# MrBottleTree/fake-video-detection-engine

Hardware: NVIDIA B200
Metric: 1080p_keyframes_per_sec_v5_ela_texture (higher is better)
Workload: dtype int32

## Files before the change

### fake-video-detection-engine_b200/csrc/v5ela_device.cuh

```cuda
#pragma once
#include <stdint.h>
#include <string.h>

#include "v5ela.h"

#ifdef __CUDACC__
#define V5_DEV __device__ __forceinline__
#define V5_HOSTDEV __host__ __device__ __forceinline__
#else
#define V5_DEV inline
#define V5_HOSTDEV inline
#endif

#ifndef V5_NS
#define V5_NS v5
#endif

namespace v5plan {

#ifndef V5_NT
#define V5_NT 256
#endif
#ifndef V5_TW_MAX
#define V5_TW_MAX 30
// ... 460 lines not shown
V5_DEV int neg_cr_of(const uint32_t *w, int k)
{
    return rgb_dot<false, -32768, 27439, 5329>(w, k, 65535 - ((128 << 16) + 32767)) >> 16;
}

template <bool WANT_Y, bool WANT_C>
V5_DEV void convert8x2(const uint8_t *la, const uint8_t *lb, U2 &y0, U2 &y1, uint32_t &cbo, uint32_t &cro)
{
    uint32_t a[6], b[6];
#pragma unroll
    for (int i = 0; i < 3; i++) {
        const U2 ta = reinterpret_cast<const U2 *>(la)[i], tb = reinterpret_cast<const U2 *>(lb)[i];
        a[2 * i] = ta.x; a[2 * i + 1] = ta.y;
        b[2 * i] = tb.x; b[2 * i + 1] = tb.y;
    }
    if (WANT_Y) {
        int ya[8], yb[8];
#pragma unroll
        for (int k = 0; k < 8; k++) {
            ya[k] = y_of(a, k);
            yb[k] = y_of(b, k);
        }
        y0 = U2{pack4sat(ya[0], ya[1], ya[2], ya[3]), pack4sat(ya[4], ya[5], ya[6], ya[7])};
        y1 = U2{pack4sat(yb[0], yb[1], yb[2], yb[3]), pack4sat(yb[4], yb[5], yb[6], yb[7])};
    }
    if (WANT_C) {
        int c[4], d[4];
#pragma unroll
        for (int j = 0; j < 4; j++) {
            const int bias = 1 + (j & 1);
            c[j] = (bias - (neg_cb_of(a, 2 * j) + neg_cb_of(a, 2 * j + 1) + neg_cb_of(b, 2 * j) + neg_cb_of(b, 2 * j + 1))) >> 2;
            d[j] = (bias - (neg_cr_of(a, 2 * j) + neg_cr_of(a, 2 * j + 1) + neg_cr_of(b, 2 * j) + neg_cr_of(b, 2 * j + 1))) >> 2;
        }
        cbo = pack4sat(c[0], c[1], c[2], c[3]);
        cro = pack4sat(d[0], d[1], d[2], d[3]);
    }
}

V5_DEV void convert_wait_done(int tid, Smem &S, const KParams &p, const Geo &g, int r, ThreadAcc &acc, bool prefetch_next)
{
    mbar_wait(reinterpret_cast<uint64_t *>(&S.done_bar), (acc.phase >> 2) & 1u);
    acc.phase ^= 4u;
    if (prefetch_next) stage_prefetch(tid, S, p, g, r + 1);
}

V5_DEV void stage_convert(int tid, Smem &S, const KParams &p, const Geo &g, int r, ThreadAcc &acc, bool defer, bool prefetch_next, bool copy_carry = true)
{
    const int last_cline = ((g.h + 1) >> 1) - 1 - 8 * r;
    const int last_line = g.h - 1 - 16 * r;
    const uint8_t(*src)[RGB_PITCH] = S.rgb[rb(r)];
    bool waiting = defer;
    if (RGB_BUFS == 2 && !waiting && copy_carry)
        for (int i = tid; i < RGB_PITCH / 16; i += NT)
            reinterpret_cast<U4 *>(S.rgb_carry[r & 1])[i] = reinterpret_cast<const U4 *>(src[15])[i];
#if defined(V5_CONVERT_UNROLL) && V5_CONVERT_UNROLL
#pragma unroll 2
#endif
    for (int u = tid; u < 8 * 2 * BAND_MCUS; u += NT) {
        const int li = u / (2 * BAND_MCUS), ox = u - li * (2 * BAND_MCUS);
        const int mcu = g.m0 - 1 + (ox >> 1);
        if (ox >= 2 * g.band_mcus || mcu < 0 || mcu >= g.mw) continue;
        U2 y0, y1;
        uint32_t cb, cr;
        convert8x2<true, true>(&src[2 * li][24 * ox], &src[2 * li + 1][24 * ox], y0, y1, cb, cr);
        const int jc = li < last_cline ? li : last_cline;
        int lb = 2 * jc + 1;
        if (lb > last_line) lb = last_line;
        if (jc != li || lb != 2 * li + 1) {
            U2 d0, d1;
            convert8x2<false, true>(&src[2 * jc][24 * ox], &src[lb][24 * ox], d0, d1, cb, cr);
        }
        if (waiting) {
            convert_wait_done(tid, S, p, g, r, acc, prefetch_next);
            waiting = false;
            if (RGB_BUFS == 2)
                for (int i = tid; i < RGB_PITCH / 16; i += NT)
                    reinterpret_cast<U4 *>(S.rgb_carry[r & 1])[i] = reinterpret_cast<const U4 *>(src[15])[i];
        }
        *reinterpret_cast<U2 *>(&S.yorig[ring16(r, 2 * li)][8 * ox]) = y0;
        *reinterpret_cast<U2 *>(&S.yorig[ring16(r, 2 * li + 1)][8 * ox]) = y1;
        *reinterpret_cast<uint32_t *>(&S.cenc[0][li][4 * ox]) = cb;
        *reinterpret_cast<uint32_t *>(&S.cenc[1][li][4 * ox]) = cr;
    }
    if (waiting) {
        convert_wait_done(tid, S, p, g, r, acc, prefetch_next);
        if (RGB_BUFS == 2)
            for (int i = tid; i < RGB_PITCH / 16; i += NT)
                reinterpret_cast<U4 *>(S.rgb_carry[r & 1])[i] = reinterpret_cast<const U4 *>(src[15])[i];
    }
}

V5_DEV void stage_carries(int tid, Smem &S, int r, bool has_band)
{
    constexpr int NRGB = RGB_PITCH / 16, NY = Y_PITCH / 16;
    if (tid < NRGB) {
        if (has_band) reinterpret_cast<U4 *>(S.rgb_carry[r & 1])[tid] = reinterpret_cast<const U4 *>(S.rgb[rb(r)][15])[tid];
    } else if (FUSE2_OK && tid < NRGB + 2 * NY) {
        const int k = tid - NRGB, line = k >= NY ? 1 : 0, i = k - line * NY;
        reinterpret_cast<U4 *>(S.ycarry[FUSE2_OK ? line : 0])[FUSE2_OK ? i : 0] = reinterpret_cast<const U4 *>(S.yorig[ring16(r - 1, 14 + line)])[i];
    }
}

#define V5_C0_298 2446
#define V5_C0_390 3196
#define V5_C0_541 4433
#define V5_C0_765 6270
#define V5_C0_899 7373
#define V5_C1_175 9633
#define V5_C1_501 12299
#define V5_C1_847 15137
#define V5_C1_961 16069
#define V5_C2_053 16819
#define V5_C2_562 20995
#define V5_C3_072 25172

template <int S, bool PASS1>
V5_DEV void fdct8(int *v)
{
    const int n = PASS1 ? 11 : 15, rnd = 1 << (n - 1);
    const int t0 = v[0] + v[7 * S], t7 = v[0] - v[7 * S], t1 = v[S] + v[6 * S], t6 = v[S] - v[6 * S];
    const int t2 = v[2 * S] + v[5 * S], t5 = v[2 * S] - v[5 * S], t3 = v[3 * S] + v[4 * S], t4 = v[3 * S] - v[4 * S];
    const int t10 = t0 + t3, t13 = t0 - t3, t11 = t1 + t2, t12 = t1 - t2;
    if (PASS1) {
        v[0] = (t10 + t11 - 1024) * 4;
        v[4 * S] = (t10 - t11) * 4;
    } else {
        v[0] = (t10 + t11 + 2) >> 2;
        v[4 * S] = (t10 - t11 + 2) >> 2;
    }
    v[2 * S] = (t12 * V5_C0_541 + t13 * (V5_C0_541 + V5_C0_765) + rnd) >> n;
    v[6 * S] = (t13 * V5_C0_541 + t12 * (V5_C0_541 - V5_C1_847) + rnd) >> n;
    const int z1 = (t4 + t7) * -V5_C0_899, z2 = (t5 + t6) * -V5_C2_562;
    const int z3 = t4 + t6, z4 = t5 + t7;
    const int z5 = (z3 + z4) * V5_C1_175 + rnd;
    const int z3b = z3 * -V5_C1_961 + z5, z4b = z4 * -V5_C0_390 + z5;
    v[7 * S] = (t4 * V5_C0_298 + z1 + z3b) >> n;
    v[5 * S] = (t5 * V5_C2_053 + z2 + z4b) >> n;
    v[3 * S] = (t6 * V5_C3_072 + z2 + z3b) >> n;
    v[S] = (t7 * V5_C1_501 + z1 + z4b) >> n;
}

template <int S, bool FINAL>
V5_DEV void idct8(int *v)
{
    const int n = FINAL ? 18 : 11;
    const int rnd = (1 << (n - 1)) + (FINAL ? (128 << 18) : 0);
    const int i2 = v[2 * S], i6 = v[6 * S];
    const int t2 = i2 * V5_C0_541 + i6 * (V5_C0_541 - V5_C1_847);
    const int t3 = i6 * V5_C0_541 + i2 * (V5_C0_541 + V5_C0_765);
    const int t0 = (v[0] + v[4 * S]) * 8192 + rnd, t1 = (v[0] - v[4 * S]) * 8192 + rnd;
    int u0 = v[7 * S], u1 = v[5 * S], u2 = v[3 * S], u3 = v[S];
    const int z1 = (u0 + u3) * -V5_C0_899, z2 = (u1 + u2) * -V5_C2_562;
    const int z3 = u0 + u2, z4 = u1 + u3;
    const int z5 = (z3 + z4) * V5_C1_175;
    const int z3b = z3 * -V5_C1_961 + z5, z4b = z4 * -V5_C0_390 + z5;
    u0 = u0 * V5_C0_298 + z1 + z3b;
    u1 = u1 * V5_C2_053 + z2 + z4b;
    u2 = u2 * V5_C3_072 + z2 + z3b;
    u3 = u3 * V5_C1_501 + z1 + z4b;
    v[0] = (t0 + t3 + u3) >> n;
    v[7 * S] = (t0 + t3 - u3) >> n;
    v[S] = (t1 + t2 + u2) >> n;
    v[6 * S] = (t1 + t2 - u2) >> n;
    v[2 * S] = (t1 - t2 + u1) >> n;
    v[5 * S] = (t1 - t2 - u1) >> n;
    v[3 * S] = (t0 - t3 + u0) >> n;
    v[4 * S] = (t0 - t3 - u0) >> n;
}

V5_DEV uint32_t pack_s16(int lo, int hi)
{
#ifndef __CUDACC__
    if (lo < -32768 || lo > 32767 || hi < -32768 || hi > 32767) range_violations()++;
#endif
    return prmt((uint32_t)lo, (uint32_t)hi, 0x5410u);
}
V5_DEV int s16_lo(uint32_t w) { return (int)prmt(w, 0u, 0x9910u); }
V5_DEV int s16_hi(uint32_t w) { return (int)w >> 16; }

#if !V5_MMA_BLOCKS
struct BlockTask {
    const QEntry *q;
    const uint8_t *in;
    uint8_t *out;
    int pitch;
    bool active;
};

template <bool FAST>
V5_DEV BlockTask block_task(int blk, Smem &S, const KParams &p, const Geo &g, int r, bool want_y)
{
    BlockTask t;
    t.active = false;
    t.q = S.qtab[0];
    t.in = nullptr;
    t.out = nullptr;
    t.pitch = 0;
    const int tw = g.m1 - g.m0;
    const int nl = want_y ? 4 * tw : 0;
    if (blk < nl) {
        const int br = blk >= 2 * tw ? 1 : 0, bc = blk - br * 2 * tw;
        if (16 * r + 8 * br >= g.h || (!FAST && 16 * g.m0 + 8 * bc >= g.w)) return t;
        const int row = ring16(r, 8 * br), col = 16 + 8 * bc;
        t.in = &S.yorig[row][col];
        t.out = &S.ydec[ringd(r, 8 * br)][col];
        t.pitch = Y_PITCH;
        t.active = true;
    } else {
        const int c = blk - nl;
        if (c >= 2 * g.band_mcus) return t;
        const int comp = c >= g.band_mcus ? 1 : 0, cbk = c - comp * g.band_mcus;
        const int mcu = g.m0 - 1 + cbk;
        if (mcu < 0 || mcu >= g.mw) return t;
        t.q = S.qtab[1];
        t.in = &S.cenc[comp][0][8 * cbk];
        t.out = &S.cdec[comp][ring8(r, 0)][8 * cbk];
        t.pitch = C_PITCH;
        t.active = true;
    }
    return t;
}

template <bool FAST>
V5_DEV BlockTask block_task_of(int tid, Smem &S, const KParams &p, const Geo &g, int r, bool want_y, int round)
{
    return block_task<FAST>(round * (NT / 4) + (tid >> 5) * 8 + ((tid & 31) >> 2), S, p, g, r, want_y);
}

V5_DEV int blocks_in_band(const Geo &g, bool want_y) { return (want_y ? 4 * (g.m1 - g.m0) : 0) + 2 * g.band_mcus; }


V5_DEV void blocks_rows_fwd(int tid, Smem &S, const BlockTask &t)
{
    const int warp = tid >> 5, lane = tid & 31, j = lane & 3, bw = lane >> 2;
    if (!t.active) return;
    int a[8], b[8];
    const U2 wa = *reinterpret_cast<const U2 *>(t.in + (2 * j) * t.pitch);
    const U2 wb = *reinterpret_cast<const U2 *>(t.in + (2 * j + 1) * t.pitch);
#pragma unroll
    for (int k = 0; k < 4; k++) {
        a[k] = (int)byte_of(wa.x, k); a[4 + k] = (int)byte_of(wa.y, k);
        b[k] = (int)byte_of(wb.x, k); b[4 + k] = (int)byte_of(wb.y, k);
    }
    fdct8<1, true>(a);
    fdct8<1, true>(b);
    uint32_t *ts = &S.tscratch[warp][36 * bw];
#pragma unroll
    for (int c = 0; c < 8; c++) ts[4 * c + j] = pack_s16(a[c], b[c]);
}

V5_DEV void blocks_cols(int tid, Smem &S, const BlockTask &t, int *col)
{
    const int warp = tid >> 5, lane = tid & 31, j = lane & 3, bw = lane >> 2;
    if (!t.active) return;
    const uint32_t *ts = &S.tscratch[warp][36 * bw];
    const U4 w0 = *reinterpret_cast<const U4 *>(ts + 8 * j), w1 = *reinterpret_cast<const U4 *>(ts + 8 * j + 4);
    int a[8] = {s16_lo(w0.x), s16_hi(w0.x), s16_lo(w0.y), s16_hi(w0.y), s16_lo(w0.z), s16_hi(w0.z), s16_lo(w0.w), s16_hi(w0.w)};
    int b[8] = {s16_lo(w1.x), s16_hi(w1.x), s16_lo(w1.y), s16_hi(w1.y), s16_lo(w1.z), s16_hi(w1.z), s16_lo(w1.w), s16_hi(w1.w)};
    fdct8<1, false>(a);
    fdct8<1, false>(b);
    const QEntry *qj = t.q + 2 * j;
#pragma unroll
    for (int k = 0; k < 8; k++) {
        const QEntry ea = qj[8 * k], eb = qj[8 * k + 1];
        const uint32_t xa = (uint32_t)(a[k] + (a[k] >> 31) + ea.bias), xb = (uint32_t)(b[k] + (b[k] >> 31) + eb.bias);
        a[k] = (int)umulhi32(xa, ea.recip) * ea.t - ea.unbias;
        b[k] = (int)umulhi32(xb, eb.recip) * eb.t - eb.unbias;
    }
    idct8<1, false>(a);
    idct8<1, false>(b);
#pragma unroll
    for (int k = 0; k < 8; k++) {
        col[k] = a[k];
        col[8 + k] = b[k];
    }
}

V5_DEV void blocks_cols_store(int tid, Smem &S, const BlockTask &t, const int *col)
{
    const int warp = tid >> 5, lane = tid & 31, j = lane & 3, bw = lane >> 2;
    if (!t.active) return;
    uint32_t *rs = &S.tscratch[warp][36 * bw];
#pragma unroll
    for (int k = 0; k < 8; k++) rs[4 * k + j] = pack_s16(col[k], col[8 + k]);
}

V5_DEV void blocks_rows_inv(int tid, Smem &S, const BlockTask &t)
{
    const int warp = tid >> 5, lane = tid & 31, j = lane & 3, bw = lane >> 2;
    if (!t.active) return;
    const uint32_t *rs = &S.tscratch[warp][36 * bw];
    const U4 w0 = *reinterpret_cast<const U4 *>(rs + 8 * j), w1 = *reinterpret_cast<const U4 *>(rs + 8 * j + 4);
    int a[8] = {s16_lo(w0.x), s16_hi(w0.x), s16_lo(w0.y), s16_hi(w0.y), s16_lo(w0.z), s16_hi(w0.z), s16_lo(w0.w), s16_hi(w0.w)};
    int b[8] = {s16_lo(w1.x), s16_hi(w1.x), s16_lo(w1.y), s16_hi(w1.y), s16_lo(w1.z), s16_hi(w1.z), s16_lo(w1.w), s16_hi(w1.w)};
    idct8<1, true>(a);
    idct8<1, true>(b);
    *reinterpret_cast<U2 *>(t.out + (2 * j) * t.pitch) = U2{pack4sat(a[0], a[1], a[2], a[3]), pack4sat(a[4], a[5], a[6], a[7])};
    *reinterpret_cast<U2 *>(t.out + (2 * j + 1) * t.pitch) = U2{pack4sat(b[0], b[1], b[2], b[3]), pack4sat(b[4], b[5], b[6], b[7])};
}

#else
constexpr int MMA_NP = V5_MMA_NP;

template <int PITCH, bool ALL_ACTIVE>
V5_DEV void blocks_section(int tid, const mma::LaneConsts *K, const uint8_t *in, uint8_t *out, const QEntry *q, int npairs, int act_lo,
                           int act_hi)
{
    const int warp = tid >> 5;
    for (int k0 = warp * MMA_NP; k0 < npairs; k0 += (NT / 32) * MMA_NP) {
        mma::PairTask t[MMA_NP];
#pragma unroll
        for (int j = 0; j < MMA_NP; j++) {
            const int k = k0 + j < npairs ? k0 + j : npairs - 1;
            t[j].in = in + 16 * k;
            t[j].out = out + 16 * k;
            t[j].q = q;
            t[j].ipitch = t[j].opitch = PITCH;
            t[j].left = k0 + j < npairs && (ALL_ACTIVE || (2 * k >= act_lo && 2 * k < act_hi));
            t[j].right = k0 + j < npairs && (ALL_ACTIVE || (2 * k + 1 >= act_lo && 2 * k + 1 < act_hi));
        }
#ifdef __CUDA_ARCH__
        mma::dct_pairs<MMA_NP>(t, *K, tid & 31);
#else
        for (int j = 0; j < MMA_NP; j++)
            if (t[j].left || t[j].right) mma::dct_pair_emu(t[j], K);
#endif
    }
}

template <bool FAST>
V5_DEV void stage_blocks_mma(int tid, Smem &S, const KParams &p, const Geo &g, int r, bool want_y)
{
    const int tw = g.m1 - g.m0;
#ifdef __CUDA_ARCH__
    mma::LaneConsts Kreg;
#pragma unroll
    for (int j = 0; j < 8; j++) reinterpret_cast<U4 *>(&Kreg)[j] = S.lane[j][tid & 31];
    const mma::LaneConsts *K = &Kreg;
#else
    const mma::LaneConsts *K = S.lane;
#endif
    if (want_y) {
        int hi = 2 * tw;
        if (!FAST) {
            const int inside = (g.w - 16 * g.m0 + 7) >> 3;
            hi = inside < hi ? inside : hi;
        }
#pragma unroll 1
        for (int br = 0; br < 2; br++) {
            if (16 * r + 8 * br >= g.h) break;
            blocks_section<Y_PITCH, FAST>(tid, K, &S.yorig[ring16(r, 8 * br)][16], &S.ydec[ringd(r, 8 * br)][16], S.qtab[0], tw, 0, hi);
        }
    }
    const int lo = g.m0 == 0 ? 1 : 0;
    const int hi = g.band_mcus < g.mw - g.m0 + 1 ? g.band_mcus : g.mw - g.m0 + 1;
#pragma unroll 1
    for (int comp = 0; comp < 2; comp++)
        blocks_section<C_PITCH, false>(tid, K, &S.cenc[comp][0][0], &S.cdec[comp][ring8(r, 0)][0], S.qtab[1], (g.band_mcus + 1) >> 1, lo, hi);
}
#endif

V5_DEV void upsample8(const uint8_t *lc, const uint8_t *ln, int gcx0, int wc1, bool fancy, int out[8])
{
    const uint32_t c0 = *reinterpret_cast<const uint32_t *>(lc - 4), n0 = *reinterpret_cast<const uint32_t *>(ln - 4);
    const uint32_t c1 = *reinterpret_cast<const uint32_t *>(lc), n1 = *reinterpret_cast<const uint32_t *>(ln);
    const uint32_t c2 = *reinterpret_cast<const uint32_t *>(lc + 4), n2 = *reinterpret_cast<const uint32_t *>(ln + 4);
    if (!fancy) {
#pragma unroll
        for (int j = 0; j < 4; j++) out[2 * j] = out[2 * j + 1] = (int)byte_of(c1, j) - 128;
        return;
    }
    int cs[6];
    cs[0] = dp4a_us(c0, sel_const(SEL_THREE + 3), dp4a_us(n0, sel_const(SEL_ONE + 3), 0));
#pragma unroll
    for (int j = 0; j < 4; j++) cs[1 + j] = dp4a_us(c1, sel_const(SEL_THREE + j), dp4a_us(n1, sel_const(SEL_ONE + j), 0));
    cs[5] = dp4a_us(c2, sel_const(SEL_THREE), dp4a_us(n2, sel_const(SEL_ONE), 0));
    if (gcx0 == 0) cs[0] = cs[1];
    if (gcx0 + 4 > wc1) {
#pragma unroll
        for (int j = 1; j < 6; j++)
            if (gcx0 + j - 1 > wc1) cs[j] = cs[j - 1];
    }
#pragma unroll
    for (int j = 0; j < 4; j++) {
        const int t3 = 3 * cs[j + 1] + (8 - 2048);
        out[2 * j] = (t3 + cs[j]) >> 4;
        out[2 * j + 1] = (t3 + cs[j + 2] - 1) >> 4;
    }
}

V5_DEV void upsample8_fast(const uint8_t *lc, const uint8_t *ln, bool left_edge, bool right_edge, int out[8])
{
    const uint32_t c0 = *reinterpret_cast<const uint32_t *>(lc - 4), n0 = *reinterpret_cast<const uint32_t *>(ln - 4);
    const uint32_t c1 = *reinterpret_cast<const uint32_t *>(lc), n1 = *reinterpret_cast<const uint32_t *>(ln);
    const uint32_t c2 = *reinterpret_cast<const uint32_t *>(lc + 4), n2 = *reinterpret_cast<const uint32_t *>(ln + 4);
    const uint32_t cs = left_edge ? prmt(c1, 0u, 0x2100u) : prmt(c0, c1, 0x6543u), ns = left_edge ? prmt(n1, 0u, 0x2100u) : prmt(n0, n1, 0x6543u);
    const uint32_t ce = right_edge ? prmt(c1, 0u, 0x3321u) : prmt(c1, c2, 0x4321u), ne = right_edge ? prmt(n1, 0u, 0x3321u) : prmt(n1, n2, 0x4321u);
    uint32_t w[5];
    w[0] = prmt(cs, ns, 0x5140u);
    w[1] = prmt(c1, n1, 0x5140u);
    w[2] = prmt(c1, n1, 0x6251u);
    w[3] = prmt(c1, n1, 0x7362u);
    w[4] = prmt(ce, ne, 0x7362u);
    const uint32_t ke = sel_const(SEL_TRI), ko = sel_const(SEL_TRI + 1);
#pragma unroll
    for (int j = 0; j < 4; j++) {
        out[2 * j] = dp4a_us(w[j], ke, 8 - 2048) >> 4;
        out[2 * j + 1] = dp4a_us(w[j + 1], ko, 7 - 2048) >> 4;
    }
}

template <bool FAST, bool TEXHIST, bool SWEEP = false>
V5_DEV void residual_row(Smem &S, const KParams &p, const Geo &g, ThreadAcc &acc, int r, int l, int ox, const int *cb, const int *cr,
                         bool ghost = false)
{
    const int y = 16 * r + l;
    const int gx0 = 16 * g.m0 + 8 * ox;
    const int col = 16 + 8 * ox;
    const int nvalid = g.w - gx0;

    const U2 yd = *reinterpret_cast<const U2 *>(&S.ydec[ringd(r, l)][col]);
    const uint32_t ydw[2] = {yd.x, yd.y};
    uint32_t ow[6], dw[6];
    if (RGB_BUFS == 2) {
        const uint8_t *orig = l < 0 ? &S.rgb_carry[(r - 1) & 1][3 * col] : &S.rgb[r & 1][l][3 * col];
#pragma unroll
        for (int i = 0; i < 3; i++) {
            const U2 t = reinterpret_cast<const U2 *>(orig)[i];
            ow[2 * i] = t.x; ow[2 * i + 1] = t.y;
        }
    } else {
        const uint8_t *orig = g.frame + (int64_t)y * g.row_stride + 3 * gx0;
        if (g.vec_ok && nvalid >= 8) {
#pragma unroll
            for (int i = 0; i < 3; i++) {
                const U2 t = reinterpret_cast<const U2 *>(orig)[i];
                ow[2 * i] = t.x; ow[2 * i + 1] = t.y;
            }
        } else {
            const int nb = nvalid >= 8 ? 24 : 3 * nvalid;
#pragma unroll
            for (int i = 0; i < 6; i++) {
                uint32_t w = 0;
#pragma unroll
                for (int b = 0; b < 4; b++)
                    if (4 * i + b < nb) w |= (uint32_t)orig[4 * i + b] << (8 * b);
                ow[i] = w;
            }
        }
    }
    int rec[24];
#pragma unroll
    for (int k = 0; k < 8; k++) {
        const int ykr = (int)prmt(ydw[k >> 2], sel_const(SEL_HALF), 0x4054u + ((uint32_t)(k & 3) << 8));
        const int cbv = cb[k], crv = cr[k];
        rec[3 * k] = (91881 * crv + ykr) >> 16;
        rec[3 * k + 1] = (-22554 * cbv + (-46802 * crv + ykr)) >> 16;
        rec[3 * k + 2] = (116130 * cbv + ykr) >> 16;
    }
#pragma unroll
    for (int i = 0; i < 6; i++)
        dw[i] = absdiff4(ow[i], pack4sat(rec[4 * i], rec[4 * i + 1], rec[4 * i + 2], rec[4 * i + 3]));
    if (!FAST && g.resid) {
        uint8_t *dst = g.resid + ((int64_t)y * g.w + gx0) * 3;
        if (nvalid >= 8 && g.resid_vec_ok) {
#pragma unroll
            for (int i = 0; i < 3; i++) reinterpret_cast<U2 *>(dst)[i] = U2{dw[2 * i], dw[2 * i + 1]};
        } else {
#pragma unroll
            for (int b = 0; b < 24; b++)
                if (b < 3 * nvalid) dst[b] = (uint8_t)byte_of(dw[b >> 2], b & 3);
        }
    }
    if (!FAST && nvalid < 8) {
#pragma unroll
        for (int i = 0; i < 6; i++) {
            const int vb = 3 * nvalid - 4 * i;
            dw[i] &= vb >= 4 ? 0xffffffffu : (vb <= 0 ? 0u : (1u << (8 * vb)) - 1u);
        }
#ifdef __CUDA_ARCH__
        atomicSub(&S.hist[0][0], (uint32_t)(8 - nvalid));
        atomicSub(&S.hist[1][0], (uint32_t)(8 - nvalid));
        atomicSub(&S.hist[2][0], (uint32_t)(8 - nvalid));
#else
        S.hist[0][0] -= (uint32_t)(8 - nvalid);
        S.hist[1][0] -= (uint32_t)(8 - nvalid);
        S.hist[2][0] -= (uint32_t)(8 - nvalid);
#endif
    }
#pragma unroll
    for (int b = 0; b < 24; b++) hist_add(S.hist[b % 3], dw[b >> 2], b & 3);
    if (SWEEP && ghost) {
        uint32_t sq = 0;
#pragma unroll
        for (int i = 0; i < 6; i++) sq = dp4a_uu(dw[i], dw[i], sq);
        smem_add(&S.ghost[(y >> 4) & 1][ox >> 1], sq);
    }

    int lu = l - 1, ld = l + 1;
    if (y == 0) lu = g.h > 1 ? l + 1 : l;
    if (y == g.h - 1) ld = g.h > 1 ? l - 1 : l;
    constexpr bool CARRY = FAST && FUSE2_OK;
    const uint8_t *yc = CARRY && l < 0 ? &S.ycarry[CARRY ? l + 2 : 0][CARRY ? col : 0] : &S.yorig[ring16(r, l)][col];
    const uint8_t *yu = CARRY && lu < 0 ? &S.ycarry[CARRY ? lu + 2 : 0][CARRY ? col : 0] : &S.yorig[ring16(r, lu)][col];
    const uint8_t *yd2 = CARRY && ld < 0 ? &S.ycarry[CARRY ? ld + 2 : 0][CARRY ? col : 0] : &S.yorig[ring16(r, ld)][col];
    const int wide = FAST || g.w > 1;
    uint32_t sabs = 0, ssq = 0, mx = acc.tex_maxabs;
    {
        const U2 cw = *reinterpret_cast<const U2 *>(yc);
        const U2 uw = *reinterpret_cast<const U2 *>(yu);
        const U2 lw = *reinterpret_cast<const U2 *>(yd2);
        const int edge = !FAST && nvalid < 8 ? nvalid - 1 : -1;
        const int nacc = edge >= 0 ? edge : 8;
        const uint32_t hl = gx0 == 0 ? yc[wide] : yc[-1], hr = nvalid == 8 ? yc[6] : yc[8];
        const uint32_t x[3] = {prmt(hl, cw.x, 0x6540u), prmt(cw.x, cw.y, 0x6543u), prmt(cw.y, hr, 0x7743u)};
        const uint32_t ud[2][2] = {{uw.x, lw.x}, {uw.y, lw.y}};
#pragma unroll
        for (int k = 0; k < 8; k++) {
            const int w0 = k >> 2, s0 = k & 3;
            int lap = dp4a_us(ud[w0][0], sel_const(SEL_ONE + s0), dp4a_us(ud[w0][1], sel_const(SEL_ONE + s0), 0));
            if (s0 <= 1) {
                lap = dp4a_us(x[w0], sel_const(SEL_LAP + s0), lap);
            } else if (s0 == 2) {
                lap = dp4a_us(x[w0 + 1], sel_const(SEL_ONE), dp4a_us(x[w0], sel_const(SEL_LAP + 2), lap));
            } else {
                lap = dp4a_us(x[w0 + 1], sel_const(SEL_LAP + 3), dp4a_us(x[w0], sel_const(SEL_ONE + 3), lap));
            }
            lap = lap < 0 ? -lap : lap;
            if (FAST || k < nacc) {
                sabs += (uint32_t)lap;
                ssq += (uint32_t)(lap * lap);
                mx = (uint32_t)lap > mx ? (uint32_t)lap : mx;
                if (TEXHIST) smem_inc(&S.tex_hist[lap < 255 ? lap : 255]);
            }
        }
        if (!FAST && edge >= 0) {
            const int ctr = yc[edge];
            const int side = wide ? (edge == 0 && gx0 == 0 ? ctr : (int)yc[edge - 1]) : ctr;
            int lap = 2 * side + (int)yu[edge] + (int)yd2[edge] - 4 * ctr;
            lap = lap < 0 ? -lap : lap;
            sabs += (uint32_t)lap;
            ssq += (uint32_t)(lap * lap);
            mx = (uint32_t)lap > mx ? (uint32_t)lap : mx;
            if (TEXHIST) smem_inc(&S.tex_hist[lap < 255 ? lap : 255]);
        }
    }
    acc.tex_sumabs += sabs;
    acc.tex_sumsq += ssq;
    acc.tex_maxabs = mx;
}

template <bool FAST, bool TEXHIST, bool SWEEP = false>
V5_DEV void residual_unit(Smem &S, const KParams &p, const Geo &g, ThreadAcc &acc, int r, int l, int ox, bool ghost = false)
{
    const int y = 16 * r + l;
    const int gx0 = 16 * g.m0 + 8 * ox;
    const int col = 16 + 8 * ox;

    const int hc1 = ((g.h + 1) >> 1) - 1, wc1 = ((g.w + 1) >> 1) - 1;
    const int crow = y >> 1;
    int nrow = (y & 1) ? crow + 1 : crow - 1;
    nrow = nrow < 0 ? 0 : (nrow > hc1 ? hc1 : nrow);
    const int lcur = ring8(r, crow - 8 * r), lnb = ring8(r, nrow - 8 * r);
    const int ccol = col >> 1, gcx0 = gx0 >> 1;
    const bool fancy = wc1 > 1;
    int cb[8], cr[8];
    if (FAST) {
        upsample8_fast(&S.cdec[0][lcur][ccol], &S.cdec[0][lnb][ccol], gcx0 == 0, gcx0 + 4 > wc1, cb);
        upsample8_fast(&S.cdec[1][lcur][ccol], &S.cdec[1][lnb][ccol], gcx0 == 0, gcx0 + 4 > wc1, cr);
    } else {
        upsample8(&S.cdec[0][lcur][ccol], &S.cdec[0][lnb][ccol], gcx0, wc1, fancy, cb);
        upsample8(&S.cdec[1][lcur][ccol], &S.cdec[1][lnb][ccol], gcx0, wc1, fancy, cr);
    }

    residual_row<FAST, TEXHIST, SWEEP>(S, p, g, acc, r, l, ox, cb, cr, ghost);
}

V5_DEV void chroma_pairs(const uint8_t *la, const uint8_t *lb, bool left_edge, bool right_edge, uint32_t w[5])
{
    const uint32_t a0 = *reinterpret_cast<const uint32_t *>(la - 4), b0 = *reinterpret_cast<const uint32_t *>(lb - 4);
    const uint32_t a1 = *reinterpret_cast<const uint32_t *>(la), b1 = *reinterpret_cast<const uint32_t *>(lb);
    const uint32_t a2 = *reinterpret_cast<const uint32_t *>(la + 4), b2 = *reinterpret_cast<const uint32_t *>(lb + 4);
    const uint32_t as = left_edge ? prmt(a1, 0u, 0x2100u) : prmt(a0, a1, 0x6543u), bs = left_edge ? prmt(b1, 0u, 0x2100u) : prmt(b0, b1, 0x6543u);
    const uint32_t ae = right_edge ? prmt(a1, 0u, 0x3321u) : prmt(a1, a2, 0x4321u), be = right_edge ? prmt(b1, 0u, 0x3321u) : prmt(b1, b2, 0x4321u);
    w[0] = prmt(as, bs, 0x5140u);
    w[1] = prmt(a1, b1, 0x5140u);
    w[2] = prmt(a1, b1, 0x6251u);
    w[3] = prmt(a1, b1, 0x7362u);
    w[4] = prmt(ae, be, 0x7362u);
}

template <bool TEXHIST>
V5_DEV void residual_pair(Smem &S, const KParams &p, const Geo &g, ThreadAcc &acc, int r, int pi, int ox, bool v0, bool v1)
{
    const int col = 16 + 8 * ox, ccol = col >> 1, gcx0 = (16 * g.m0 + 8 * ox) >> 1;
    const int hc1 = ((g.h + 1) >> 1) - 1, wc1 = (g.w >> 1) - 1;
    int ja = pi - 1, jb = pi;
    if (8 * r + ja < 0) ja = jb;
    if (8 * r + jb > hc1) jb = ja;
    const bool le = gcx0 == 0, re = gcx0 + 4 > wc1;
    uint32_t wb[5], wr[5];
    chroma_pairs(&S.cdec[0][ring8(r, ja)][ccol], &S.cdec[0][ring8(r, jb)][ccol], le, re, wb);
    chroma_pairs(&S.cdec[1][ring8(r, ja)][ccol], &S.cdec[1][ring8(r, jb)][ccol], le, re, wr);
#if !defined(V5_PAIR_UNROLL) || V5_PAIR_UNROLL
#pragma unroll
#else
#pragma unroll 1
#endif
    for (int h = 0; h < 2; h++) {
        if (!(h ? v1 : v0)) continue;
        const uint32_t ke = sel_const(SEL_TRI + 2 * h), ko = sel_const(SEL_TRI + 2 * h + 1);
        int cb[8], cr[8];
#pragma unroll
        for (int j = 0; j < 4; j++) {
            cb[2 * j] = dp4a_us(wb[j], ke, 8 - 2048) >> 4;
            cb[2 * j + 1] = dp4a_us(wb[j + 1], ko, 7 - 2048) >> 4;
            cr[2 * j] = dp4a_us(wr[j], ke, 8 - 2048) >> 4;
            cr[2 * j + 1] = dp4a_us(wr[j + 1], ko, 7 - 2048) >> 4;
        }
        residual_row<true, TEXHIST>(S, p, g, acc, r, 2 * pi - 1 + h, ox, cb, cr);
    }
}

template <bool TEXHIST>
V5_DEV void stage_residual_pairs(int tid, Smem &S, const KParams &p, const Geo &g, ThreadAcc &acc, int r)
{
    const int n8 = 2 * (g.m1 - g.m0);
    const uint32_t inv = 65536u / (uint32_t)n8 + 1u;
    const int ylo = 16 * g.r0, yhi = 16 * g.r1 < g.h ? 16 * g.r1 : g.h;
    for (int u = tid; u < 8 * n8; u += NT) {
        const int pi = (int)(((uint32_t)u * inv) >> 16), ox = u - pi * n8;
        const int y0 = 16 * r + 2 * pi - 1;
        const bool v0 = y0 >= ylo && y0 < yhi, v1 = y0 + 1 >= ylo && y0 + 1 < yhi;
        if (!v0 && !v1) continue;
        residual_pair<TEXHIST>(S, p, g, acc, r, pi, ox, v0, v1);
    }
}

template <bool FAST, bool TEXHIST, bool SWEEP = false>
V5_DEV void stage_residual(int tid, Smem &S, const KParams &p, const Geo &g, ThreadAcc &acc, int r, bool ghost = false)
{
    const int n8 = 2 * (g.m1 - g.m0);
    const uint32_t inv = 65536u / (uint32_t)n8 + 1u;
    const int ylo = 16 * g.r0, yhi = 16 * g.r1 < g.h ? 16 * g.r1 : g.h;
    for (int u = tid; u < 16 * n8; u += NT) {
        const int wl = (int)(((uint32_t)u * inv) >> 16), ox = u - wl * n8;
        const int l = wl - 1, y = 16 * r + l;
        if (y < ylo || y >= yhi || (!FAST && 16 * g.m0 + 8 * ox >= g.w)) continue;
        residual_unit<FAST, TEXHIST, SWEEP>(S, p, g, acc, r, l, ox, ghost);
    }
}

template <bool RAGGED>
V5_DEV void make_geo(const KParams &p, int work, Geo &g, int &frame)
{
    uint32_t rem, n_strips, n_segs;
    if (RAGGED) {
        int lo = 0, hi = p.n - 1;
        while (lo < hi) {
            const int mid = (lo + hi + 1) >> 1;
            if (p.frames[mid].work_base <= (uint32_t)work) lo = mid;
            else hi = mid - 1;
        }
        frame = lo;
        const FrameDesc &d = p.frames[lo];
        rem = (uint32_t)work - d.work_base;
        n_strips = (uint32_t)d.n_strips;
        n_segs = (uint32_t)d.n_segs;
        g.h = d.h; g.w = d.w; g.mw = d.mw; g.mh = d.mh;
        g.row_stride = d.row_stride;
        g.vec_ok = (int)(d.flags & 1u);
        g.resid_vec_ok = (int)((d.flags >> 1) & 1u);
        g.frame = d.rgb;
        g.resid = d.resid;
    } else {
        n_strips = (uint32_t)p.n_strips;
        if (work < p.work_split) {
            n_segs = (uint32_t)p.n_segs;
            const uint32_t per_frame = n_strips * n_segs;
            frame = (int)((uint32_t)work / per_frame);
            rem = (uint32_t)work - (uint32_t)frame * per_frame;
        } else {
            n_segs = (uint32_t)p.n_segs_b;
            const uint32_t per_frame = n_strips * n_segs, w2 = (uint32_t)(work - p.work_split);
            const uint32_t f2 = w2 / per_frame;
            frame = p.split_frame + (int)f2;
            rem = w2 - f2 * per_frame;
        }
        g.h = p.h; g.w = p.w; g.mw = p.mw; g.mh = p.mh;
        g.row_stride = p.row_stride;
        g.vec_ok = p.vec_ok;
        g.resid_vec_ok = p.resid_vec_ok;
        g.frame = p.rgb + (int64_t)frame * p.frame_stride;
        g.resid = p.residual ? p.residual + (int64_t)frame * p.h * p.w * 3 : nullptr;
    }
    const uint32_t seg = rem / n_strips, strip = rem - seg * n_strips;
    g.m0 = (int)((strip * (uint32_t)g.mw) / n_strips);
    g.m1 = (int)(((strip + 1) * (uint32_t)g.mw) / n_strips);
    g.r0 = (int)((seg * (uint32_t)g.mh) / n_segs);
    g.r1 = (int)(((seg + 1) * (uint32_t)g.mh) / n_segs);
    g.xb0 = 16 * (g.m0 - 1);
    g.band_mcus = g.m1 - g.m0 + 2;
}


}
```

### fake-video-detection-engine_b200/csrc/v5ela_workitem.cuh

```cuda
#pragma once
#include "v5ela_device.cuh"

namespace V5_NS {

#ifdef __CUDA_ARCH__
#define V5_BLOCK_TASK(t) const BlockTask t = block_task_of<FAST>((int)threadIdx.x, S, p, g, r, want_y, round);
#define V5_GET_TASK(t) (void)0
#define V5_FOR_WARP(...)                     \
    {                                        \
        const int tid = (int)threadIdx.x;    \
        ThreadAcc &acc = acc_store[0];       \
        (void)acc;                           \
        __VA_ARGS__;                         \
    }                                        \
    __syncwarp();
#define V5_FOR_THREADS(...)                  \
    {                                        \
        const int tid = (int)threadIdx.x;    \
        ThreadAcc &acc = acc_store[0];       \
        (void)acc;                           \
        (void)tid;                           \
        __VA_ARGS__;                         \
    }                                        \
    __syncthreads();
#define V5_FOR_THREADS_NOSYNC(...)           \
    {                                        \
        const int tid = (int)threadIdx.x;    \
        ThreadAcc &acc = acc_store[0];       \
        (void)acc;                           \
        __VA_ARGS__;                         \
    }
#define V5_FOR_EACH_WARP(...)                \
    {                                        \
        const int tid = (int)threadIdx.x;    \
        __VA_ARGS__;                         \
    }                                        \
    __syncthreads();
#else
#if defined(V5_EMU_REVERSE) && V5_EMU_REVERSE
#define V5_EMU_TID_LOOP(step) for (int tid = NT - (step); tid >= 0; tid -= (step))
#else
#define V5_EMU_TID_LOOP(step) for (int tid = 0; tid < NT; tid += (step))
#endif
#define V5_FOR_EACH_WARP(...)                        \
    V5_EMU_TID_LOOP(32) {                            \
        __VA_ARGS__;                                 \
    }
#define V5_FOR_THREADS_NOSYNC(...) V5_FOR_THREADS(__VA_ARGS__)
#define V5_BLOCK_TASK(t)
#define V5_GET_TASK(t) const BlockTask t = block_task_of<FAST>(tid, S, p, g, r, want_y, round)
#define V5_FOR_WARP(...)                     \
    V5_EMU_TID_LOOP(1) {                     \
        ThreadAcc &acc = acc_store[tid];     \
        (void)acc;                           \
        __VA_ARGS__;                         \
    }
#define V5_FOR_THREADS(...)                  \
    V5_EMU_TID_LOOP(1) {                     \
        ThreadAcc &acc = acc_store[tid];     \
        (void)acc;                           \
        __VA_ARGS__;                         \
    }
#endif

#ifdef __CUDA_ARCH__
V5_DEV void flush_partials(int tid, Smem &S, ThreadAcc &acc)
{
    unsigned long long sq = acc.tex_sumsq, sa = acc.tex_sumabs;
    uint32_t mx = acc.tex_maxabs;
#pragma unroll
    for (int o = 16; o > 0; o >>= 1) {
        sq += __shfl_xor_sync(0xffffffffu, sq, o);
        sa += __shfl_xor_sync(0xffffffffu, sa, o);
        mx = max(mx, __shfl_xor_sync(0xffffffffu, mx, o));
    }
    if ((tid & 31) == 0) {
        atomicAdd(&S.tex_sumsq, sq);
        atomicAdd(&S.tex_sumabs, sa);
        atomicMax(&S.tex_maxabs, mx);
    }
}
V5_DEV void flush_global(int tid, Smem &S, v5ela_record *rec, uint32_t *tex_hist)
{
    for (int i = tid; i < 3 * 256; i += NT) {
        const uint32_t c = (&S.hist[0][0])[i];
        if (c) atomicAdd(&rec->ela_hist[0][0] + i, c);
    }
    if (tex_hist)
        for (int i = tid; i < 256; i += NT) {
            const uint32_t c = S.tex_hist[i];
            if (c) atomicAdd(tex_hist + i, c);
        }
    if (tid == 0) {
        atomicAdd(reinterpret_cast<unsigned long long *>(&rec->tex_sumabs), S.tex_sumabs);
        atomicAdd(reinterpret_cast<unsigned long long *>(&rec->tex_sumsq), S.tex_sumsq);
        atomicMax(reinterpret_cast<uint32_t *>(&rec->tex_maxabs), S.tex_maxabs);
    }
}
#else
inline void flush_partials(int, Smem &S, ThreadAcc &acc)
{
    S.tex_sumsq += acc.tex_sumsq;
    S.tex_sumabs += acc.tex_sumabs;
    if (acc.tex_maxabs > S.tex_maxabs) S.tex_maxabs = acc.tex_maxabs;
}
inline void flush_global(int tid, Smem &S, v5ela_record *rec, uint32_t *tex_hist)
{
    for (int i = tid; i < 3 * 256; i += NT) (&rec->ela_hist[0][0])[i] += (&S.hist[0][0])[i];
    if (tex_hist)
        for (int i = tid; i < 256; i += NT) tex_hist[i] += S.tex_hist[i];
    if (tid == 0) {
        rec->tex_sumabs += S.tex_sumabs;
        rec->tex_sumsq += S.tex_sumsq;
        if (S.tex_maxabs > rec->tex_maxabs) rec->tex_maxabs = (uint16_t)S.tex_maxabs;
    }
}
#endif

V5_DEV void flush_ghost_row(int tid, Smem &S, const Geo &g, uint32_t *ghost, int R)
{
    for (int c = tid; c < g.m1 - g.m0; c += NT) {
        ghost[(int64_t)R * g.mw + g.m0 + c] = S.ghost[R & 1][c];
        S.ghost[R & 1][c] = 0;
    }
}

template <bool FAST, bool TEXHIST, bool RAGGED = false, bool SWEEP = false>
V5_DEV void process_work_item(Smem &S, const KParams &p, int work, ThreadAcc *acc_store)
{
    static_assert(!RAGGED || (!FAST && !TEXHIST), "ragged batches take the general instantiation");
    static_assert(!SWEEP || RAGGED, "a sweep is a ragged batch");
    Geo g;
    int frame;
    make_geo<RAGGED>(p, work, g, frame);
    const SweepEntry *const entry = SWEEP ? sweep_entries(p.frames, p.n) + frame : nullptr;
    const QuantTab *const sweep_q = SWEEP ? sweep_quant(p.frames, p.n) + 2 * entry->slot : nullptr;
    uint32_t *const ghost = SWEEP ? entry->ghost : nullptr;

    V5_FOR_THREADS({
        for (int i = tid; i < 3 * 256; i += NT) (&S.hist[0][0])[i] = 0;
        if (TEXHIST)
            for (int i = tid; i < 256; i += NT) S.tex_hist[i] = 0;
        if (SWEEP)
            for (int i = tid; i < 2 * TW_MAX; i += NT) (&S.ghost[0][0])[i] = 0;
        for (int i = tid; i < 2 * 64; i += NT) {
            const QuantTab &q = SWEEP ? sweep_q[i >> 6] : p.q[i >> 6];
            const int k = i & 63;
#if V5_MMA_BLOCKS
            S.qtab[i >> 6][mma::qswz_pos(k)] = mma::qswz_entry(q.recip[k], q.bias[k], q.t[k], q.unbias[k]);
#else
            S.qtab[i >> 6][k] = QEntry{q.recip[k], q.bias[k], q.t[k], q.unbias[k]};
#endif
        }
#if V5_MMA_BLOCKS
#ifdef __CUDA_ARCH__
        for (int i = tid; i < 32 * 8; i += NT) S.lane[i & 7][i >> 3] = reinterpret_cast<const U4 *>(p.lane_consts)[i];
#else
        for (int i = tid; i < 32 * (int)(sizeof(mma::LaneConsts) / 16); i += NT)
            reinterpret_cast<U4 *>(S.lane)[i] = reinterpret_cast<const U4 *>(p.lane_consts)[i];
#endif
#endif
        if (tid == 0) {
            S.tex_sumabs = 0;
            S.tex_sumsq = 0;
            S.tex_maxabs = 0;
        }
        acc.tex_sumabs = 0;
        acc.tex_sumsq = 0;
        acc.tex_maxabs = 0;
    })

    const int r_first = g.r0 > 0 ? g.r0 - 1 : 0;
    const bool bulk = FAST || use_bulk(p, g);
    const bool rest = !FAST && load_rest_needed(p, g, bulk);
    V5_FOR_THREADS(if (bulk) stage_prefetch(tid, S, p, g, r_first))
#ifndef V5_SPLIT_BARRIER
#define V5_SPLIT_BARRIER 0
#endif
    constexpr bool SPLIT = FAST && RGB_BUFS == 2 && V5_SPLIT_BARRIER;
#ifndef V5_PAIR_ROWS
#define V5_PAIR_ROWS 1
#endif
    constexpr bool PAIRS = FAST && V5_PAIR_ROWS;
    constexpr bool FUSE = FAST && FUSE2_OK;
    static_assert(!FUSE || (PAIRS && NT >= RGB_PITCH / 16 + 2 * (Y_PITCH / 16)), "two-phase band loop: pairs, and one thread per carried 16 bytes");
    if (FUSE) {
        int pend = -1;
        for (int r = r_first; r <= g.r1; r++) {
            const bool has_band = r < g.mh;
            const bool want_y = r >= g.r0 && r < g.r1;
            const bool next_band = r + 1 <= g.r1 && r + 1 < g.mh;
            if (!has_band && 16 * r - 1 >= g.h) break;
            V5_FOR_THREADS({
                if (pend >= 0) stage_residual_pairs<TEXHIST>(tid, S, p, g, acc, pend);
                if (has_band) {
                    mbar_wait(reinterpret_cast<uint64_t *>(&S.full_bar[rb(r)]), (acc.phase >> rb(r)) & 1u);
                    acc.phase ^= 1u << rb(r);
                    stage_convert(tid, S, p, g, r, acc, false, false, false);
                }
            })
            pend = r;
            V5_FOR_THREADS_NOSYNC({
                if (next_band) stage_prefetch(tid, S, p, g, r + 1);
                stage_carries(tid, S, r, has_band);
            })
            if (has_band) {
#if V5_MMA_BLOCKS
                V5_FOR_EACH_WARP(stage_blocks_mma<FAST>(tid, S, p, g, r, want_y))
#else
                const int rounds = (blocks_in_band(g, want_y) + NT / 4 - 1) / (NT / 4);
                for (int round = 0; round < rounds; round++) {
                    V5_BLOCK_TASK(t)
                    V5_FOR_WARP(V5_GET_TASK(t); blocks_rows_fwd(tid, S, t))
                    V5_FOR_WARP(V5_GET_TASK(t); blocks_cols(tid, S, t, acc.col))
                    V5_FOR_WARP(V5_GET_TASK(t); blocks_cols_store(tid, S, t, acc.col))
                    V5_FOR_WARP(V5_GET_TASK(t); blocks_rows_inv(tid, S, t))
                }
                V5_FOR_THREADS((void)0)
#endif
            } else {
                V5_FOR_THREADS((void)0)
            }
        }
        if (pend >= 0) {
            V5_FOR_THREADS(stage_residual_pairs<TEXHIST>(tid, S, p, g, acc, pend))
        }
    } else {
        bool pending = false;
        for (int r = r_first; r <= g.r1; r++) {
            const bool has_band = r < g.mh;
            const bool want_y = r >= g.r0 && r < g.r1;
            const bool next_band = r + 1 <= g.r1 && r + 1 < g.mh;
            if (!has_band && 16 * r - 1 >= g.h) break;
            if (has_band) {
                if (rest) {
                    V5_FOR_THREADS(stage_load_rest(tid, S, p, g, r, bulk))
                }
                V5_FOR_THREADS({
                    const bool defer = SPLIT && pending;
                    if (!defer && RGB_BUFS == 2 && bulk && next_band) stage_prefetch(tid, S, p, g, r + 1);
                    if (bulk) {
                        mbar_wait(reinterpret_cast<uint64_t *>(&S.full_bar[rb(r)]), (acc.phase >> rb(r)) & 1u);
                        acc.phase ^= 1u << rb(r);
                    }
                    stage_convert(tid, S, p, g, r, acc, defer, defer && bulk && next_band);
                })
                pending = false;
                if (RGB_BUFS == 1 && bulk && next_band) {
                    V5_FOR_WARP(stage_prefetch(tid, S, p, g, r + 1))
                }
#if V5_MMA_BLOCKS
                V5_FOR_EACH_WARP(stage_blocks_mma<FAST>(tid, S, p, g, r, want_y))
#else
                const int rounds = (blocks_in_band(g, want_y) + NT / 4 - 1) / (NT / 4);
                for (int round = 0; round < rounds; round++) {
                    V5_BLOCK_TASK(t)
                    V5_FOR_WARP(V5_GET_TASK(t); blocks_rows_fwd(tid, S, t))
                    V5_FOR_WARP(V5_GET_TASK(t); blocks_cols(tid, S, t, acc.col))
                    V5_FOR_WARP(V5_GET_TASK(t); blocks_cols_store(tid, S, t, acc.col))
                    V5_FOR_WARP(V5_GET_TASK(t); blocks_rows_inv(tid, S, t))
                }
                V5_FOR_THREADS((void)0)
#endif
            }
            if (SPLIT && next_band) {
                V5_FOR_THREADS_NOSYNC({
                    if (PAIRS) stage_residual_pairs<TEXHIST>(tid, S, p, g, acc, r);
                    else stage_residual<FAST, TEXHIST>(tid, S, p, g, acc, r);
                    mbar_arrive(reinterpret_cast<uint64_t *>(&S.done_bar));
                })
                pending = true;
            } else {
                V5_FOR_THREADS(if (PAIRS) stage_residual_pairs<TEXHIST>(tid, S, p, g, acc, r); else stage_residual<FAST, TEXHIST, SWEEP>(tid, S, p, g, acc, r, ghost != nullptr))
            }
            if (SWEEP && ghost && r - 1 >= g.r0 && r < g.r1) {
                V5_FOR_THREADS(flush_ghost_row(tid, S, g, ghost, r - 1))
            }
        }
    }

    V5_FOR_THREADS(flush_partials(tid, S, acc); if (SWEEP && ghost) flush_ghost_row(tid, S, g, ghost, g.r1 - 1))
    V5_FOR_THREADS(flush_global(tid, S, p.records + frame, TEXHIST ? p.tex_hist + (int64_t)frame * 256 : nullptr))
}

}
```

### include/v5ela.h

```cpp
#ifndef V5ELA_H
#define V5ELA_H

#include <stddef.h>
#include <stdint.h>

#ifdef __cplusplus
extern "C" {
#endif

#define V5ELA_ABI_VERSION 1

#if defined(__GNUC__)
#define V5ELA_API __attribute__((visibility("default")))
#else
#define V5ELA_API
#endif

typedef enum {
    V5ELA_OK = 0,
    V5ELA_ERR_INVALID = -1,
    V5ELA_ERR_CUDA = -2,
    V5ELA_ERR_NO_DEVICE = -3,
    V5ELA_ERR_NOMEM = -4,
    V5ELA_ERR_UNSUPPORTED = -5
} v5ela_status;

typedef struct v5ela_record {
    uint32_t ela_hist[3][256];
    uint64_t ela_sum[3];
    uint64_t ela_sumsq[3];
    uint64_t tex_sumabs;
    uint64_t tex_sumsq;
    uint16_t tex_maxabs;
    uint8_t  ela_max[3];
    uint8_t  pad[3];
} v5ela_record;

typedef struct v5ela_handle v5ela_handle;

V5ELA_API int         v5ela_abi_version(void);
V5ELA_API size_t      v5ela_record_bytes(void);
V5ELA_API const char *v5ela_status_string(int status);

V5ELA_API int         v5ela_create(int device, v5ela_handle **out);
V5ELA_API int         v5ela_destroy(v5ela_handle *h);
V5ELA_API const char *v5ela_last_error(const v5ela_handle *h);

V5ELA_API int v5ela_set_quality(v5ela_handle *h, int quality);
V5ELA_API int v5ela_get_quality(const v5ela_handle *h);
V5ELA_API int v5ela_get_quant_tables(const v5ela_handle *h, uint16_t luma_host[64], uint16_t chroma_host[64]);

V5ELA_API int v5ela_analyze(v5ela_handle *h, const uint8_t *d_rgb, int n, int height, int width,
                  int64_t frame_stride_bytes, int64_t row_stride_bytes,
                  void *d_records, uint8_t *d_residual, void *cuda_stream);

V5ELA_API int v5ela_analyze_ex(v5ela_handle *h, const uint8_t *d_rgb, int n, int height, int width,
                     int64_t frame_stride_bytes, int64_t row_stride_bytes,
                     void *d_records, uint8_t *d_residual, uint32_t *d_tex_hist, void *cuda_stream);

typedef struct v5ela_frame_desc {
    const uint8_t *rgb;
    int32_t height, width;
    int64_t row_stride_bytes;
    uint8_t *residual;
    uint8_t *enhanced;
} v5ela_frame_desc;
V5ELA_API int v5ela_analyze_ragged(v5ela_handle *h, const v5ela_frame_desc *frames_host, int n, void *d_records, void *cuda_stream);
V5ELA_API int v5ela_analyze_ragged_host(v5ela_handle *h, const v5ela_frame_desc *frames_host, int n, void *records_host);

V5ELA_API int v5ela_analyze_sweep(v5ela_handle *h, const v5ela_frame_desc *frames_host, int n, const int *qualities_host, int nq,
                                  void *d_records, uint32_t *d_ghost, void *cuda_stream);
V5ELA_API int v5ela_analyze_sweep_host(v5ela_handle *h, const v5ela_frame_desc *frames_host, int n, const int *qualities_host, int nq,
                                       void *records_host, uint32_t *ghost_host);

V5ELA_API int v5ela_enhance(v5ela_handle *h, const uint8_t *d_residual, const void *d_records, int n, int height, int width,
                  uint8_t *d_enhanced, void *cuda_stream);

V5ELA_API int v5ela_reduce_records(v5ela_handle *h, const void *d_records, int n, int group, void *d_out, void *cuda_stream);

V5ELA_API int v5ela_analyze_host(v5ela_handle *h, const uint8_t *rgb_host, int n, int height, int width,
                       void *records_host, uint8_t *residual_host_or_null, uint8_t *enhanced_host_or_null,
                       void *cuda_stream);

V5ELA_API int v5ela_spectrum(v5ela_handle *h, const uint8_t *d_gray, int n, int height, int width,
                   int64_t frame_stride_bytes, int64_t row_stride_bytes, uint8_t *d_out, void *cuda_stream);
V5ELA_API int v5ela_spectrum_host(v5ela_handle *h, const uint8_t *gray_host, int n, int height, int width,
                        uint8_t *out_host);

typedef struct v5ela_gray_desc {
    const uint8_t *gray;
    int32_t height, width;
    int64_t row_stride_bytes;
    uint8_t *out;
} v5ela_gray_desc;
V5ELA_API int v5ela_spectrum_ragged(v5ela_handle *h, const v5ela_gray_desc *frames_host, int n, void *cuda_stream);
V5ELA_API int v5ela_spectrum_ragged_host(v5ela_handle *h, const v5ela_gray_desc *frames_host, int n);

V5ELA_API int64_t v5ela_jpeg_bound(int height, int width, int channels);
V5ELA_API int v5ela_jpeg_encode(v5ela_handle *h, const uint8_t *d_img, int n, int height, int width, int channels,
                      int64_t frame_stride_bytes, int64_t row_stride_bytes, int quality,
                      uint8_t *d_out, int64_t out_stride_bytes, int32_t *d_sizes, void *cuda_stream);
V5ELA_API int v5ela_jpeg_encode_host(v5ela_handle *h, const uint8_t *img_host, int n, int height, int width, int channels,
                           int quality, uint8_t *out_host, int64_t out_stride_bytes, int32_t *sizes_host);

V5ELA_API int v5ela_jpeg_info(const uint8_t *file_host, int64_t len, int *height, int *width, int *channels);
V5ELA_API int v5ela_jpeg_info_batch(const uint8_t *const *files_host, const int64_t *lens, int n, int32_t *dims_out, int *bad_index);
V5ELA_API int v5ela_jpeg_decode(v5ela_handle *h, const uint8_t *const *files_host, const int64_t *lens, int n,
                      uint8_t *d_rgb, const int64_t *rgb_offsets, uint8_t *d_gray, const int64_t *gray_offsets,
                      int32_t *d_status, void *cuda_stream);
V5ELA_API int v5ela_jpeg_decode_host(v5ela_handle *h, const uint8_t *const *files_host, const int64_t *lens, int n,
                           uint8_t *rgb_host, const int64_t *rgb_offsets, uint8_t *gray_host, const int64_t *gray_offsets);

V5ELA_API int v5ela_profile_enable(v5ela_handle *h, int enable);
V5ELA_API int v5ela_profile_read(v5ela_handle *h, double *fused_ms_sum, int64_t *fused_launches, int reset);

#define V5ELA_INST_GENERAL 0
#define V5ELA_INST_FAST 1
#define V5ELA_INST_TEXHIST 2
V5ELA_API int v5ela_last_instantiation(const v5ela_handle *h);

#define V5ELA_BLOCKS_SMEM 0
#define V5ELA_BLOCKS_MMA 1
#define V5ELA_BLOCKS_DEFAULT V5ELA_BLOCKS_SMEM
V5ELA_API int v5ela_set_block_stage(v5ela_handle *h, int mode);
V5ELA_API int v5ela_get_block_stage(const v5ela_handle *h);

V5ELA_API int64_t v5ela_launch_count(const v5ela_handle *h);

#ifdef __cplusplus
}
#endif
#endif
```

Baseline: 117,100.

## Fuse Laplacian texture stats into MMA block stage and default to MMA blocks

Moves the Laplacian texture-statistics computation into the MMA DCT block stage for the first 8-row half of each band. Each lane computes a texture unit alongside the tensor-core DCT pairs, and a separate pass handles the band's last row. The per-pixel path then returns early and skips its texture work on the FAST MMA path. It also switches the default block stage from shared-memory DCT to the MMA path, which changes the instruction mix and register pressure, and it adds a profiling script.

New measurement: 120,400, median of 6. 2.9% higher.

```diff
diff --git a/fake-video-detection-engine_b200/csrc/v5ela_device.cuh b/fake-video-detection-engine_b200/csrc/v5ela_device.cuh
--- a/fake-video-detection-engine_b200/csrc/v5ela_device.cuh
+++ b/fake-video-detection-engine_b200/csrc/v5ela_device.cuh
@@ -786,11 +786,72 @@
 #else
 constexpr int MMA_NP = V5_MMA_NP;
 
-template <int PITCH, bool ALL_ACTIVE>
+struct TexRow {
+    const uint8_t *yc, *yu, *yd;
+    bool valid;
+};
+
+V5_DEV TexRow tex_row(const Smem &S, const Geo &g, int r, int l)
+{
+    const int y = 16 * r + l, yhi = 16 * g.r1 < g.h ? 16 * g.r1 : g.h;
+    int lu = l - 1, ld = l + 1;
+    if (y == 0) lu = g.h > 1 ? l + 1 : l;
+    if (y == g.h - 1) ld = g.h > 1 ? l - 1 : l;
+    return TexRow{&S.yorig[ring16(r, l)][16], &S.yorig[ring16(r, lu)][16], &S.yorig[ring16(r, ld)][16], y >= 16 * g.r0 && y < yhi};
+}
+
+V5_DEV void tex_unit(const Smem &S, const Geo &g, ThreadAcc &acc, const TexRow &t, int x, bool valid)
+{
+    const int gx0 = 16 * g.m0 + x;
+    const uint8_t *yc = t.yc + x;
+    const U2 cw = *reinterpret_cast<const U2 *>(yc);
+    const U2 uw = *reinterpret_cast<const U2 *>(t.yu + x);
+    const U2 lw = *reinterpret_cast<const U2 *>(t.yd + x);
+    const uint32_t hl = gx0 == 0 ? yc[1] : yc[-1], hr = gx0 + 8 == g.w ? yc[6] : yc[8];
+    const uint32_t e[3] = {prmt(hl, cw.x, 0x6540u), prmt(cw.x, cw.y, 0x6543u), prmt(cw.y, hr, 0x7743u)};
+    const uint32_t ud[2][2] = {{uw.x, lw.x}, {uw.y, lw.y}};
+    uint32_t sabs = 0, ssq = 0, mx = acc.tex_maxabs;
+#pragma unroll
+    for (int k = 0; k < 8; k++) {
+        const int w0 = k >> 2, s0 = k & 3;
+        int lap = dp4a_us(ud[w0][0], sel_const(SEL_ONE + s0), dp4a_us(ud[w0][1], sel_const(SEL_ONE + s0), 0));
+        if (s0 <= 1) {
+            lap = dp4a_us(e[w0], sel_const(SEL_LAP + s0), lap);
+        } else if (s0 == 2) {
+            lap = dp4a_us(e[w0 + 1], sel_const(SEL_ONE), dp4a_us(e[w0], sel_const(SEL_LAP + 2), lap));
+        } else {
+            lap = dp4a_us(e[w0 + 1], sel_const(SEL_LAP + 3), dp4a_us(e[w0], sel_const(SEL_ONE + 3), lap));
+        }
+        lap = lap < 0 ? -lap : lap;
+        sabs += (uint32_t)lap;
+        ssq += (uint32_t)(lap * lap);
+        mx = (uint32_t)lap > mx ? (uint32_t)lap : mx;
+    }
+    valid = valid && t.valid;
+    acc.tex_sumabs += valid ? sabs : 0u;
+    acc.tex_sumsq += valid ? ssq : 0u;
+    acc.tex_maxabs = valid ? mx : acc.tex_maxabs;
+}
+
+V5_DEV ThreadAcc &acc_of(ThreadAcc *acc_store, int tid)
+{
+#ifdef __CUDA_ARCH__
+    (void)tid;
+    return acc_store[0];
+#else
+    return acc_store[tid];
+#endif
+}
+
+template <int PITCH, bool ALL_ACTIVE, bool TEX = false>
 V5_DEV void blocks_section(int tid, const mma::LaneConsts *K, const uint8_t *in, uint8_t *out, const QEntry *q, int npairs, int act_lo,
-                           int act_hi)
+                           int act_hi, Smem *S = nullptr, const Geo *g = nullptr, int r = 0, ThreadAcc *acc_store = nullptr)
 {
     const int warp = tid >> 5;
+#ifdef __CUDA_ARCH__
+    TexRow tr;
+    if (TEX) tr = tex_row(*S, *g, r, ((tid & 31) >> 1) - 1);
+#endif
     for (int k0 = warp * MMA_NP; k0 < npairs; k0 += (NT / 32) * MMA_NP) {
         mma::PairTask t[MMA_NP];
 #pragma unroll
@@ -804,16 +865,25 @@
             t[j].right = k0 + j < npairs && (ALL_ACTIVE || (2 * k + 1 >= act_lo && 2 * k + 1 < act_hi));
         }
 #ifdef __CUDA_ARCH__
+        if (TEX)
+#pragma unroll
+            for (int j = 0; j < MMA_NP; j++)
+                tex_unit(*S, *g, acc_store[0], tr, 16 * (k0 + j < npairs ? k0 + j : npairs - 1) + 8 * (tid & 1), k0 + j < npairs);
         mma::dct_pairs<MMA_NP>(t, *K, tid & 31);
 #else
         for (int j = 0; j < MMA_NP; j++)
             if (t[j].left || t[j].right) mma::dct_pair_emu(t[j], K);
+        if (TEX)
+            for (int lane = 0; lane < 32; lane++)
+                for (int j = 0; j < MMA_NP; j++)
+                    tex_unit(*S, *g, acc_store[tid + lane], tex_row(*S, *g, r, (lane >> 1) - 1),
+                             16 * (k0 + j < npairs ? k0 + j : npairs - 1) + 8 * (lane & 1), k0 + j < npairs);
 #endif
     }
 }
 
 template <bool FAST>
-V5_DEV void stage_blocks_mma(int tid, Smem &S, const KParams &p, const Geo &g, int r, bool want_y)
+V5_DEV void stage_blocks_mma(int tid, Smem &S, const KParams &p, const Geo &g, int r, bool want_y, ThreadAcc *acc_store)
 {
     const int tw = g.m1 - g.m0;
 #ifdef __CUDA_ARCH__
@@ -830,8 +900,11 @@
             const int inside = (g.w - 16 * g.m0 + 7) >> 3;
             hi = inside < hi ? inside : hi;
         }
+        if (FAST)
+            blocks_section<Y_PITCH, true, true>(tid, K, &S.yorig[ring16(r, 0)][16], &S.ydec[ringd(r, 0)][16], S.qtab[0], tw, 0, hi, &S, &g, r,
+                                                acc_store);
 #pragma unroll 1
-        for (int br = 0; br < 2; br++) {
+        for (int br = FAST ? 1 : 0; br < 2; br++) {
             if (16 * r + 8 * br >= g.h) break;
             blocks_section<Y_PITCH, FAST>(tid, K, &S.yorig[ring16(r, 8 * br)][16], &S.ydec[ringd(r, 8 * br)][16], S.qtab[0], tw, 0, hi);
         }
@@ -841,6 +914,18 @@
 #pragma unroll 1
     for (int comp = 0; comp < 2; comp++)
         blocks_section<C_PITCH, false>(tid, K, &S.cenc[comp][0][0], &S.cdec[comp][ring8(r, 0)][0], S.qtab[1], (g.band_mcus + 1) >> 1, lo, hi);
+    if (FAST) {
+        const int l = want_y ? 15 : -1, y = 16 * r + l;
+        if (l < 0 || y == g.h - 1) {
+#ifdef __CUDA_ARCH__
+            const int t0 = tid, t1 = tid + 1;
+#else
+            const int t0 = tid, t1 = tid + 32;
+#endif
+            for (int t = t0; t < t1; t++)
+                for (int u = t; u < 2 * tw; u += NT) tex_unit(S, g, acc_of(acc_store, t), tex_row(S, g, r, l), 8 * u, true);
+        }
+    }
 }
 #endif
 
@@ -981,6 +1066,7 @@
         smem_add(&S.ghost[(y >> 4) & 1][ox >> 1], sq);
     }
 
+    if (FAST && V5_MMA_BLOCKS) return;
     int lu = l - 1, ld = l + 1;
     if (y == 0) lu = g.h > 1 ? l + 1 : l;
     if (y == g.h - 1) ld = g.h > 1 ? l - 1 : l;
diff --git a/fake-video-detection-engine_b200/csrc/v5ela_workitem.cuh b/fake-video-detection-engine_b200/csrc/v5ela_workitem.cuh
--- a/fake-video-detection-engine_b200/csrc/v5ela_workitem.cuh
+++ b/fake-video-detection-engine_b200/csrc/v5ela_workitem.cuh
@@ -206,7 +206,7 @@
             })
             if (has_band) {
 #if V5_MMA_BLOCKS
-                V5_FOR_EACH_WARP(stage_blocks_mma<FAST>(tid, S, p, g, r, want_y))
+                V5_FOR_EACH_WARP(stage_blocks_mma<FAST>(tid, S, p, g, r, want_y, acc_store))
 #else
                 const int rounds = (blocks_in_band(g, want_y) + NT / 4 - 1) / (NT / 4);
                 for (int round = 0; round < rounds; round++) {
@@ -250,7 +250,7 @@
                     V5_FOR_WARP(stage_prefetch(tid, S, p, g, r + 1))
                 }
 #if V5_MMA_BLOCKS
-                V5_FOR_EACH_WARP(stage_blocks_mma<FAST>(tid, S, p, g, r, want_y))
+                V5_FOR_EACH_WARP(stage_blocks_mma<FAST>(tid, S, p, g, r, want_y, acc_store))
 #else
                 const int rounds = (blocks_in_band(g, want_y) + NT / 4 - 1) / (NT / 4);
                 for (int round = 0; round < rounds; round++) {
diff --git a/include/v5ela.h b/include/v5ela.h
--- a/include/v5ela.h
+++ b/include/v5ela.h
@@ -121,7 +121,7 @@
 
 #define V5ELA_BLOCKS_SMEM 0
 #define V5ELA_BLOCKS_MMA 1
-#define V5ELA_BLOCKS_DEFAULT V5ELA_BLOCKS_SMEM
+#define V5ELA_BLOCKS_DEFAULT V5ELA_BLOCKS_MMA
 V5ELA_API int v5ela_set_block_stage(v5ela_handle *h, int mode);
 V5ELA_API int v5ela_get_block_stage(const v5ela_handle *h);
 
diff --git a/profiles/r03/stage_perf.py b/profiles/r03/stage_perf.py
--- /dev/null
+++ b/profiles/r03/stage_perf.py
@@ -0,0 +1,38 @@
+import json
+import os
+import sys
+
+ROOT = sys.argv[1] if len(sys.argv) > 1 else os.path.dirname(os.path.dirname(os.path.dirname(os.path.abspath(__file__))))
+sys.path.insert(0, os.path.join(ROOT, "fake-video-detection-engine_b200"))
+import torch
+import v5ela
+from v5ela.batch import get_handle
+
+CASES = [(256, 1080, 1920, True), (256, 1080, 1920, False), (64, 2160, 3840, False), (576, 720, 1280, False)]
+
+
+def rate(n, h, w, residual, iters=20):
+    t = v5ela.gen_batch_torch(0, n, h, w, 0)
+    recs = torch.empty((n, 3144), dtype=torch.uint8, device="cuda")
+    res = torch.empty_like(t) if residual else None
+    for _ in range(3):
+        v5ela.analyze_batch(t, want_residual=residual, records_out=recs, residual_out=res)
+    torch.cuda.synchronize()
+    e0, e1 = torch.cuda.Event(enable_timing=True), torch.cuda.Event(enable_timing=True)
+    e0.record()
+    for _ in range(iters):
+        v5ela.analyze_batch(t, want_residual=residual, records_out=recs, residual_out=res)
+    e1.record()
+    torch.cuda.synchronize()
+    ms = e0.elapsed_time(e1) / iters
+    return ms, n / ms * 1e3
+
+
+if __name__ == "__main__":
+    hd = get_handle(torch.cuda.current_device())
+    for stage in ("smem", "mma"):
+        hd.block_stage = stage
+        for n, h, w, residual in CASES:
+            ms, fps = rate(n, h, w, residual)
+            print(json.dumps({"root": ROOT, "stage": stage, "n": n, "h": h, "w": w, "residual": residual,
+                              "instantiation": hd.last_instantiation, "ms": round(ms, 4), "frames_per_s": round(fps, 1)}), flush=True)
```
